# fegennari/3DWorld

Measured on NVIDIA H100. Metric: height cells/s @8192^2 8-octave domain-warp, higher is better.
Workload: dtype f32

## Files before the change

### 3dworld_b200/csrc/tw_heightgen.cu

```cuda
#include "tw_internal.h"
#include <unordered_map>
#include <vector>
#include <algorithm>
#include "tw_noise.cuh"
#include "tw_noise2.cuh"
#include <stdlib.h>

namespace {

constexpr int F_TABLE = TW_F_TABLE_SIZE;

__device__ __forceinline__ float sinf_lut(const float *__restrict__ tab, float v) {
	return (v < 0.0f) ? -__ldg(tab + (tw_x86_f2i(TW_SSCALE*(-v))&(TW_TSIZE-1))) : __ldg(tab + (tw_x86_f2i(TW_SSCALE*v)&(TW_TSIZE-1)));
}
__device__ __forceinline__ float cosf_lut(const float *__restrict__ tab, float v) {
	return __ldg(tab + TW_TSIZE + (tw_x86_f2i(TW_SSCALE*fabsf(v))&(TW_TSIZE-1)));
}
__device__ __forceinline__ float smin(float a, float b) {return (b < a) ? b : a;}
__device__ __forceinline__ float smax(float a, float b) {return (a < b) ? b : a;}

struct PostParams {
	tw_hmap_params h;
	int   shape;
	int   need_postproc;
// ... 68 lines not shown
	int   gen_shape;
	float4 oct[9];
	float xy_scale;
	float hmap_scale;
	float freq_last, rsum_last;
};

template<bool SIMPLEX, int SHAPE>
__device__ __forceinline__ float gen_noise(float xv, float yv, const NoiseParams &N) {
	float zval = 0.0f;
#pragma unroll 1
	for (int i = 0; i < N.octaves; ++i) {
		float4 const o = N.oct[i];
		float const px = o.x*xv + o.y, py = o.x*yv + o.z;
		float noise = SIMPLEX ? twn::simplex2(px, py) : twn::perlin2(px, py);
		if (SHAPE == 1) {noise = (float)((double)fabsf(noise) - 0.40);}
		if (SHAPE == 2) {noise = (float)(0.45 - (double)fabsf(noise));}
		zval = __fmaf_rn(o.w, noise, zval);
	}
	return zval;
}

template<bool SIMPLEX, bool WARP, int SHAPE>
__device__ __forceinline__ float get_noise_zval(float xval, float yval, const NoiseParams &N, const PostParams &P) {
	float xv = N.xy_scale*xval, yv = N.xy_scale*yval;
	if (WARP) {
		float const scale = 0.2f;
		float const dx1 = gen_noise<SIMPLEX, SHAPE>((float)((double)xv + 0.0), (float)((double)yv + 0.0), N);
		float const dy1 = gen_noise<SIMPLEX, SHAPE>((float)((double)xv + 5.2), (float)((double)yv + 1.3), N);
		float const wx = xv + scale*dx1, wy = yv + scale*dy1;
		float const dx2 = gen_noise<SIMPLEX, SHAPE>((float)((double)wx + 1.7), (float)((double)wy + 9.2), N);
		float const dy2 = gen_noise<SIMPLEX, SHAPE>((float)((double)wx + 8.3), (float)((double)wy + 2.8), N);
		xv += scale*dx2; yv += scale*dy2;
	}
	float z = gen_noise<SIMPLEX, SHAPE>(xv, yv, N);
	if (P.need_postproc) {z = postproc_noise_zval(z, P.h);}
	return z*N.hmap_scale;
}

template<bool SIMPLEX, bool WARP, int SHAPE>
__global__ void __launch_bounds__(256)
noise_grid_kernel(float *__restrict__ out, unsigned nx, unsigned ny, unsigned y_off, float mx0_single, float my0_single, const float2 *__restrict__ tile_origins,
	NoiseParams N, PostParams P, const float *__restrict__ sin_tab, unsigned *__restrict__ mm)
{
	unsigned const x = blockIdx.x*blockDim.x + threadIdx.x, y = y_off + blockIdx.y*blockDim.y + threadIdx.y, tile = blockIdx.z;
	float mx0 = mx0_single, my0 = my0_single;
	if (tile_origins) {float2 const o = __ldg(tile_origins + tile); mx0 = o.x; my0 = o.y;}
	float z = 0.0f;
	bool const valid = (x < nx && y < ny);
	if (valid) {
		float const xval = ((float)x*P.mdx + mx0)*P.dx_inv, yval = ((float)y*P.mdy + my0)*P.dy_inv;
		z = get_noise_zval<SIMPLEX, WARP, SHAPE>(xval, yval, N, P);
		float smx = 0.0f, smy = 0.0f;
		if (P.enable_glaciate && P.sine_on) {
			smx = P.sm_scale*cosf_lut(sin_tab, ((float)x*P.mdx + mx0)*P.dx_inv*P.sm_freq);
			smy = cosf_lut(sin_tab, ((float)y*P.mdy + my0)*P.dy_inv*P.sm_freq);
		}
		z = glaciate_and_bias(z, smx, smy, xval, yval, P, sin_tab);
		out[(size_t)tile*nx*ny + (size_t)y*nx + x] = z;
	}
	if (mm) {block_minmax(valid ? z : INFINITY, valid ? z : -INFINITY, mm + 2*tile);}
}

#ifndef TW_NOISE2_MIN_BLOCKS
#define TW_NOISE2_MIN_BLOCKS 2
#endif
#ifndef TW_NOISE2_PERSISTENT
#define TW_NOISE2_PERSISTENT 1
#endif
#ifndef TW_NOISE2_THREADS
#define TW_NOISE2_THREADS 512
#endif
#ifndef TW_NOISE2_BLOCK_CELLS
#define TW_NOISE2_BLOCK_CELLS 2048
#endif
static_assert(TW_NOISE2_BLOCK_CELLS % (2*TW_NOISE2_THREADS) == 0, "a block walks whole chunks of 2 cells per thread");
__device__ __forceinline__ bool noise_lattice_in_range(float2 xv, float2 yv, const NoiseParams &N) {
	float const bx = (fabsf(xv.x) + fabsf(yv.x))*N.freq_last + N.rsum_last, by = (fabsf(xv.y) + fabsf(yv.y))*N.freq_last + N.rsum_last;
	return (bx < 2097152.0f && by < 2097152.0f);
}

template<bool SIMPLEX, bool WARP> __host__ __device__ constexpr bool noise2_hash() {return SIMPLEX && WARP && TW_SIMPLEX_HASH_TABLE;}
template<bool HASH> __host__ __device__ constexpr int lut_entries() {return twn2::SIMPLEX_LUT_N + (HASH ? twn2::SIMPLEX_HASH_N : 0);}

template<bool SIMPLEX, int SHAPE, bool HASH>
__device__ __forceinline__ float2 gen_noise2(float2 xv, float2 yv, const NoiseParams &N, unsigned L) {
	float2 zval = make_float2(0.0f, 0.0f);
	if (noise_lattice_in_range(xv, yv, N)) {
#pragma unroll 1
		for (int i = 0; i < N.octaves; ++i) {
			float4 const o = N.oct[i];
			float2 const px = twn2::add2(twn2::mul2(xv, o.x), o.y), py = twn2::add2(twn2::mul2(yv, o.x), o.z);
			float2 noise = SIMPLEX ? ((TW_SIMPLEX_LUT > 0) ? twn2::simplex2_lut<HASH>(px, py, L) : twn2::simplex2(px, py)) : ((TW_SIMPLEX_LUT > 0) ? twn2::perlin2_lut(px, py, L) : twn2::perlin2(px, py));
			if (SHAPE == 1) {noise = make_float2((float)((double)fabsf(noise.x) - 0.40), (float)((double)fabsf(noise.y) - 0.40));}
			if (SHAPE == 2) {noise = make_float2((float)(0.45 - (double)fabsf(noise.x)), (float)(0.45 - (double)fabsf(noise.y)));}
			zval = twn2::fma2(noise, o.w, zval);
		}
	}
	else {zval = make_float2(gen_noise<SIMPLEX, SHAPE>(xv.x, yv.x, N), gen_noise<SIMPLEX, SHAPE>(xv.y, yv.y, N));}
	return zval;
}

#ifndef TW_NOISE2_DUAL
#define TW_NOISE2_DUAL 0
#endif
template<bool SIMPLEX, int SHAPE, bool HASH>
__device__ __forceinline__ void gen_noise2_dual(float2 xa, float2 ya, float2 xb, float2 yb, const NoiseParams &N, unsigned L, float2 &za, float2 &zb) {
	if (TW_SIMPLEX_LUT > 0 && noise_lattice_in_range(xa, ya, N) && noise_lattice_in_range(xb, yb, N)) {
		float2 zva = make_float2(0.0f, 0.0f), zvb = make_float2(0.0f, 0.0f);
#pragma unroll 1
		for (int i = 0; i < N.octaves; ++i) {
			float4 const o = N.oct[i];
			float const f = o.x, rx = o.y, ry = o.z, mag = o.w;
			float2 const pxa = twn2::add2(twn2::mul2(xa, f), rx), pya = twn2::add2(twn2::mul2(ya, f), ry);
			float2 const pxb = twn2::add2(twn2::mul2(xb, f), rx), pyb = twn2::add2(twn2::mul2(yb, f), ry);
			float2 na = SIMPLEX ? twn2::simplex2_lut<HASH>(pxa, pya, L) : twn2::perlin2_lut(pxa, pya, L);
			float2 nb = SIMPLEX ? twn2::simplex2_lut<HASH>(pxb, pyb, L) : twn2::perlin2_lut(pxb, pyb, L);
			if (SHAPE == 1) {na = make_float2((float)((double)fabsf(na.x) - 0.40), (float)((double)fabsf(na.y) - 0.40)); nb = make_float2((float)((double)fabsf(nb.x) - 0.40), (float)((double)fabsf(nb.y) - 0.40));}
			if (SHAPE == 2) {na = make_float2((float)(0.45 - (double)fabsf(na.x)), (float)(0.45 - (double)fabsf(na.y))); nb = make_float2((float)(0.45 - (double)fabsf(nb.x)), (float)(0.45 - (double)fabsf(nb.y)));}
			zva = twn2::fma2(na, mag, zva); zvb = twn2::fma2(nb, mag, zvb);
		}
		za = zva; zb = zvb;
	}
	else {za = gen_noise2<SIMPLEX, SHAPE, HASH>(xa, ya, N, L); zb = gen_noise2<SIMPLEX, SHAPE, HASH>(xb, yb, N, L);}
}

__device__ __forceinline__ float dadd(float a, double b) {return (float)((double)a + b);}

template<bool SIMPLEX, bool WARP, int SHAPE>
__global__ void __launch_bounds__(TW_NOISE2_THREADS, TW_NOISE2_MIN_BLOCKS)
noise_grid2_kernel(float *__restrict__ out, unsigned nx, unsigned ny, unsigned y_off, unsigned y_end, float mx0_single, float my0_single, const float2 *__restrict__ tile_origins,
	NoiseParams N, PostParams P, const float *__restrict__ sin_tab, unsigned *__restrict__ mm, const float4 *__restrict__ simplex_lut)
{
	constexpr bool HASH = noise2_hash<SIMPLEX, WARP>();
	unsigned L = 0;
	if (TW_SIMPLEX_LUT > 0) {
		extern __shared__ float4 lut_s[];
		for (int e = threadIdx.x; e < lut_entries<HASH>()*twn2::SIMPLEX_LUT_COPIES; e += blockDim.x) {lut_s[e] = __ldg(simplex_lut + e/twn2::SIMPLEX_LUT_COPIES);}
		__syncthreads();
		L = twn2::simplex_lut_base(lut_s, threadIdx.x);
		asm volatile("" : "+r"(L) :: "memory");
	}
	unsigned const tile = blockIdx.z;
	float mx0 = mx0_single, my0 = my0_single;
	if (tile_origins) {float2 const o = __ldg(tile_origins + tile); mx0 = o.x; my0 = o.y;}
	size_t const c_end = (size_t)y_end*nx;
	float lo = INFINITY, hi = -INFINITY;
	constexpr unsigned NCH = TW_NOISE2_BLOCK_CELLS/(2*TW_NOISE2_THREADS);
#pragma unroll 1
	for (unsigned grp = blockIdx.x; grp < P.ngroups; grp += gridDim.x) {
#pragma unroll 1
	for (unsigned ch = 0; ch < NCH; ++ch) {
	size_t const c0 = (size_t)y_off*nx + 2*(((size_t)grp*NCH + ch)*blockDim.x + threadIdx.x);
	unsigned y, x;
	if (c_end <= 0xffffffffull) {unsigned const c32 = (unsigned)c0; y = c32/nx; x = c32 - y*nx;}
	else {y = (unsigned)(c0/nx); x = (unsigned)(c0 - (size_t)y*nx);}
	unsigned const xb = (x + 1 < nx) ? x + 1 : 0, yb = (x + 1 < nx) ? y : y + 1;
	bool const skip = (x - P.skip_x0 < P.skip_w && y - P.skip_y0 < P.skip_h && xb - P.skip_x0 < P.skip_w && yb - P.skip_y0 < P.skip_h);
	bool const valid0 = (c0 < c_end) && !skip, valid1 = (c0 + 1 < c_end) && !skip;
	float z0 = 0.0f, z1 = 0.0f;
	if (valid0) {
		using namespace twn2;
		float2 const xs = make_float2((float)x, (float)xb), ys = make_float2((float)y, (float)yb);
		float2 const xval = mul2(add2(mul2(xs, P.mdx), mx0), P.dx_inv);
		float2 const yval = mul2(add2(mul2(ys, P.mdy), my0), P.dy_inv);
		float2 xv = mul2(xval, N.xy_scale), yv = mul2(yval, N.xy_scale);
		if (WARP) {
			float const scale = 0.2f;
			float2 dx1, dy1, dx2, dy2;
			if (TW_NOISE2_DUAL) {gen_noise2_dual<SIMPLEX, SHAPE, HASH>(make_float2(dadd(xv.x, 0.0), dadd(xv.y, 0.0)), make_float2(dadd(yv.x, 0.0), dadd(yv.y, 0.0)),
			                                                     make_float2(dadd(xv.x, 5.2), dadd(xv.y, 5.2)), make_float2(dadd(yv.x, 1.3), dadd(yv.y, 1.3)), N, L, dx1, dy1);}
			else {
				dx1 = gen_noise2<SIMPLEX, SHAPE, HASH>(make_float2(dadd(xv.x, 0.0), dadd(xv.y, 0.0)), make_float2(dadd(yv.x, 0.0), dadd(yv.y, 0.0)), N, L);
				dy1 = gen_noise2<SIMPLEX, SHAPE, HASH>(make_float2(dadd(xv.x, 5.2), dadd(xv.y, 5.2)), make_float2(dadd(yv.x, 1.3), dadd(yv.y, 1.3)), N, L);
			}
			float2 const wx = add2(xv, mul2(dx1, scale)), wy = add2(yv, mul2(dy1, scale));
			if (TW_NOISE2_DUAL) {gen_noise2_dual<SIMPLEX, SHAPE, HASH>(make_float2(dadd(wx.x, 1.7), dadd(wx.y, 1.7)), make_float2(dadd(wy.x, 9.2), dadd(wy.y, 9.2)),
			                                                     make_float2(dadd(wx.x, 8.3), dadd(wx.y, 8.3)), make_float2(dadd(wy.x, 2.8), dadd(wy.y, 2.8)), N, L, dx2, dy2);}
			else {
				dx2 = gen_noise2<SIMPLEX, SHAPE, HASH>(make_float2(dadd(wx.x, 1.7), dadd(wx.y, 1.7)), make_float2(dadd(wy.x, 9.2), dadd(wy.y, 9.2)), N, L);
				dy2 = gen_noise2<SIMPLEX, SHAPE, HASH>(make_float2(dadd(wx.x, 8.3), dadd(wx.y, 8.3)), make_float2(dadd(wy.x, 2.8), dadd(wy.y, 2.8)), N, L);
			}
			xv = add2(xv, mul2(dx2, scale)); yv = add2(yv, mul2(dy2, scale));
		}
		float2 const zz = gen_noise2<SIMPLEX, SHAPE, HASH>(xv, yv, N, L);
		z0 = zz.x; z1 = zz.y;
		if (P.need_postproc) {z0 = postproc_noise_zval(z0, P.h); z1 = postproc_noise_zval(z1, P.h);}
		z0 = z0*N.hmap_scale; z1 = z1*N.hmap_scale;
		float smx0 = 0.0f, smx1 = 0.0f, smy0 = 0.0f, smy1 = 0.0f;
		if (P.enable_glaciate && P.sine_on) {
			smx0 = P.sm_scale*cosf_lut(sin_tab, xval.x*P.sm_freq);
			smx1 = P.sm_scale*cosf_lut(sin_tab, xval.y*P.sm_freq);
			smy0 = cosf_lut(sin_tab, yval.x*P.sm_freq);
			smy1 = (yb == y) ? smy0 : cosf_lut(sin_tab, yval.y*P.sm_freq);
		}
		z0 = glaciate_and_bias(z0, smx0, smy0, xval.x, yval.x, P, sin_tab);
		z1 = glaciate_and_bias(z1, smx1, smy1, xval.y, yval.y, P, sin_tab);
		float *o = out + (size_t)(P.tile_perm ? __ldg(P.tile_perm + tile) : tile)*nx*ny + c0;
		if (valid1 && ((reinterpret_cast<size_t>(o) & 7) == 0)) {*reinterpret_cast<float2 *>(o) = make_float2(z0, z1);}
		else {o[0] = z0; if (valid1) {o[1] = z1;}}
	}
	lo = fminf(lo, fminf(valid0 ? z0 : INFINITY, valid1 ? z1 : INFINITY)); hi = fmaxf(hi, fmaxf(valid0 ? z0 : -INFINITY, valid1 ? z1 : -INFINITY));
	}
	}
	if (mm) {block_minmax(lo, hi, mm + 2*tile);}
}

template<bool SIMPLEX, bool WARP>
void launch_noise2(int shape, dim3 grid, dim3 block, cudaStream_t st, float *out, unsigned nx, unsigned ny, unsigned y_off, unsigned y_end, float mx0, float my0,
	const float2 *origins, const NoiseParams &N, const PostParams &P, const float *tab, unsigned *mm, const float4 *lut)
{
	size_t const lut_bytes = (TW_SIMPLEX_LUT > 0) ? (size_t)lut_entries<noise2_hash<SIMPLEX, WARP>()>()*twn2::SIMPLEX_LUT_COPIES*sizeof(float4) : 0;
	if (lut_bytes > 48*1024) {
		switch (shape) {
		case 1:  cudaFuncSetAttribute(noise_grid2_kernel<SIMPLEX, WARP, 1>, cudaFuncAttributeMaxDynamicSharedMemorySize, (int)lut_bytes); break;
		case 2:  cudaFuncSetAttribute(noise_grid2_kernel<SIMPLEX, WARP, 2>, cudaFuncAttributeMaxDynamicSharedMemorySize, (int)lut_bytes); break;
		default: cudaFuncSetAttribute(noise_grid2_kernel<SIMPLEX, WARP, 0>, cudaFuncAttributeMaxDynamicSharedMemorySize, (int)lut_bytes); break;
		}
	}
	switch (shape) {
	case 1:  noise_grid2_kernel<SIMPLEX, WARP, 1><<<grid, block, lut_bytes, st>>>(out, nx, ny, y_off, y_end, mx0, my0, origins, N, P, tab, mm, lut); break;
	case 2:  noise_grid2_kernel<SIMPLEX, WARP, 2><<<grid, block, lut_bytes, st>>>(out, nx, ny, y_off, y_end, mx0, my0, origins, N, P, tab, mm, lut); break;
	default: noise_grid2_kernel<SIMPLEX, WARP, 0><<<grid, block, lut_bytes, st>>>(out, nx, ny, y_off, y_end, mx0, my0, origins, N, P, tab, mm, lut); break;
	}
}

constexpr int PERLIN_LUT_OFFSET = lut_entries<true>();
__global__ void simplex_lut_kernel(float4 *__restrict__ lut) {
	int const k = blockIdx.x*blockDim.x + threadIdx.x;
	if (k < twn2::SIMPLEX_LUT_N) {lut[k] = twn2::simplex_lut_entry((float)k); lut[PERLIN_LUT_OFFSET + k] = twn2::perlin_lut_entry((float)k);}
	if (k < twn2::SIMPLEX_HASH_N) {lut[twn2::SIMPLEX_LUT_N + k] = twn2::simplex_hash_entry((float)k);}
}
static int ensure_simplex_lut(tw_ctx *ctx) {
	if (ctx->d_simplex_lut) return TW_OK;
	static_assert(twn2::SIMPLEX_HASH_N <= twn2::SIMPLEX_LUT_N, "simplex_lut_kernel's grid covers the gradient tables");
	TW_CUDA(ctx, cudaMalloc(&ctx->d_simplex_lut, (PERLIN_LUT_OFFSET + twn2::SIMPLEX_LUT_N)*sizeof(float4)));
	simplex_lut_kernel<<<(twn2::SIMPLEX_LUT_N + 127)/128, 128, 0, ctx->stream>>>((float4 *)ctx->d_simplex_lut);
	TW_LAUNCH_CHECK(ctx);
	return TW_OK;
}

struct SineTabParams {
	float msx, msy, ms2, mesh_scale_z_inv;
	float dx, dy, mx0, my0;
	int   start;
	unsigned nx, ny, xpitch, ypitch;
	int   sine_on; float sm_scale, sm_freq, dx_inv, dy_inv;
};

__global__ void sine_tables_kernel(float *__restrict__ Xt, float *__restrict__ Yt, const float *__restrict__ T, const float *__restrict__ sin_tab, SineTabParams S,
	const float *__restrict__ origins = nullptr, unsigned nux = 0, size_t xstride = 0, size_t ystride = 0)
{
	unsigned const i = blockIdx.x*blockDim.x + threadIdx.x, k = blockIdx.y;
	bool const is_y = origins ? (blockIdx.z >= nux) : (blockIdx.z != 0);
	if (origins) {
		if (is_y) {S.my0 = __ldg(origins + blockIdx.z); Yt += (size_t)(blockIdx.z - nux)*ystride;}
		else      {S.mx0 = __ldg(origins + blockIdx.z); Xt += (size_t)blockIdx.z*xstride;}
	}
	unsigned const n = is_y ? S.ny : S.nx;
	if (i >= n) return;
	if (k == F_TABLE) {
		if (!S.sine_on) return;
		if (!is_y) {Xt[(size_t)k*S.xpitch + i] = S.sm_scale*cosf_lut(sin_tab, ((float)i*S.dx + S.mx0)*S.dx_inv*S.sm_freq);}
		else       {Yt[(size_t)k*S.ypitch + i] = cosf_lut(sin_tab, ((float)i*S.dy + S.my0)*S.dy_inv*S.sm_freq);}
		return;
	}
	if ((int)k < S.start) return;
	float const *s = T + 5*k;
	if (!is_y) {
		float const x_mult = S.msx*s[4];
		float const x_const = S.ms2*s[4] + s[2] + x_mult*S.mx0;
		float const xmdx = x_mult*S.dx;
		Xt[(size_t)k*S.xpitch + i] = sinf_lut(sin_tab, xmdx*(float)i + x_const);
	}
	else {
		float const y_mult = S.msy*s[3], y_scale = S.mesh_scale_z_inv*s[0];
		float const y_const = S.ms2*s[3] + s[1] + y_mult*S.my0;
		float const ymdy = y_mult*S.dy;
		Yt[(size_t)k*S.ypitch + i] = y_scale*sinf_lut(sin_tab, ymdy*(float)i + y_const);
	}
}

constexpr int ST = 64;
constexpr int SK = 45;

__global__ void __launch_bounds__(256)
sine_grid_kernel(float *__restrict__ out, unsigned nx, unsigned ny, const float *__restrict__ Xt, const float *__restrict__ Yt,
	unsigned xpitch, unsigned ypitch, int start_ix, PostParams P, float mx0, float my0, const float *__restrict__ sin_tab, unsigned *__restrict__ mm, unsigned y_off,
	const uint2 *__restrict__ tile_tabs = nullptr, const float2 *__restrict__ tile_origins = nullptr, size_t xstride = 0, size_t ystride = 0,
	const unsigned *__restrict__ tile_perm = nullptr)
{
	__shared__ float Xs[SK][ST], Ys[SK][ST];
	if (tile_tabs) {
		unsigned const tz = tile_perm ? __ldg(tile_perm + blockIdx.z) : blockIdx.z;
		uint2 const tt = __ldg(tile_tabs + tz);
// ... 482 lines not shown
```

### 3dworld_b200/csrc/tw_noise2.cuh

```cuda
#pragma once
#include <cuda_runtime.h>
#include "tw_noise.cuh"

namespace twn2 {

typedef float2 f2;

__device__ __forceinline__ f2 splat(float v) {return make_float2(v, v);}
__device__ __forceinline__ f2 raw_fma(f2 a, f2 b, f2 c) {return make_float2(__fmaf_rn(a.x, b.x, c.x), __fmaf_rn(a.y, b.y, c.y));}
__device__ __forceinline__ f2 mul2(f2 a, f2 b) {return make_float2(__fmul_rn(a.x, b.x), __fmul_rn(a.y, b.y));}
__device__ __forceinline__ f2 mul2(f2 a, float b) {return mul2(a, splat(b));}
__device__ __forceinline__ f2 add2(f2 a, f2 b) {return make_float2(__fadd_rn(a.x, b.x), __fadd_rn(a.y, b.y));}
__device__ __forceinline__ f2 add2(f2 a, float b) {return add2(a, splat(b));}
__device__ __forceinline__ f2 sub2(f2 a, f2 b) {return make_float2(__fsub_rn(a.x, b.x), __fsub_rn(a.y, b.y));}
__device__ __forceinline__ f2 rsub2(float a, f2 b) {return sub2(splat(a), b);}
__device__ __forceinline__ f2 sumprod2(f2 a, f2 b, f2 c, f2 d) {return add2(mul2(a, b), mul2(c, d));}
__device__ __forceinline__ f2 sumprod2(f2 a, float b, f2 c, float d) {return sumprod2(a, splat(b), c, splat(d));}
__device__ __forceinline__ f2 fma2(f2 a, float b, f2 c) {return raw_fma(a, splat(b), c);}
__device__ __forceinline__ f2 fma2(f2 a, float b, float c) {return raw_fma(a, splat(b), splat(c));}
__device__ __forceinline__ f2 abs2(f2 a) {return make_float2(fabsf(a.x), fabsf(a.y));}
__device__ __forceinline__ f2 max0_2(f2 a) {return make_float2(fmaxf(a.x, 0.0f), fmaxf(a.y, 0.0f));}
__device__ __forceinline__ float rsub_max0(float a, float d) {float r; asm("sub.rn.sat.f32 %0, %1, %2;" : "=f"(r) : "f"(a), "f"(d)); return r;}
__device__ __forceinline__ f2 rsub_max0_2(float a, f2 d) {return make_float2(rsub_max0(a, d.x), rsub_max0(a, d.y));}
__device__ __forceinline__ f2 floor2(f2 x) {return make_float2(floorf(x.x), floorf(x.y));}

__device__ __forceinline__ f2 mod289(f2 x)  {f2 const t = floor2(mul2(x, 1.0f/289.0f)); return fma2(t, -289.0f, x);}
__device__ __forceinline__ f2 permute(f2 x) {return mod289(mul2(fma2(x, 34.0f, 1.0f), x));}
__device__ __forceinline__ f2 mod_int289(f2 a) {
	f2 const r = fma2(floor2(mul2(a, 1.0f/289.0f)), -289.0f, a);
	return make_float2((r.x >= 289.0f) ? r.x - 289.0f : r.x, (r.y >= 289.0f) ? r.y - 289.0f : r.y);
}
__device__ __forceinline__ f2 mod_int289_lazy(f2 a) {return fma2(floor2(mul2(a, 1.0f/289.0f)), -289.0f, a);}
__device__ __forceinline__ f2 fract2(f2 x) {return sub2(x, floor2(x));}
__device__ __forceinline__ f2 tinvsqrt(f2 r) {return rsub2(1.79284291400159f, mul2(r, 0.85373472095314f));}
__device__ __forceinline__ f2 mix2(f2 x, f2 y, f2 a) {return add2(x, mul2(a, sub2(y, x)));}
__device__ __forceinline__ f2 fade2(f2 t) {
	f2 const t3 = mul2(mul2(t, t), t);
	return mul2(t3, add2(mul2(t, add2(mul2(t, 6.0f), -15.0f)), 10.0f));
}

__device__ __forceinline__ f2 simplex2(f2 vx, f2 vy) {
	float const Cx = 0.211324865405187f, Cy = 0.366025403784439f, Cz = -0.577350269189626f, Cw = 0.024390243902439f;
	f2 const s = add2(mul2(vx, Cy), mul2(vy, Cy));
	f2 ix = floor2(add2(vx, s)), iy = floor2(add2(vy, s));
	f2 const t = add2(mul2(ix, Cx), mul2(iy, Cx));
	f2 const x0x = add2(sub2(vx, ix), t), x0y = add2(sub2(vy, iy), t);
	f2 const i1x = make_float2((x0x.x > x0y.x) ? 1.0f : 0.0f, (x0x.y > x0y.y) ? 1.0f : 0.0f);
	f2 const i1y = rsub2(1.0f, i1x);
	f2 const x12x = sub2(add2(x0x, Cx), i1x), x12y = sub2(add2(x0y, Cx), i1y), x12z = add2(x0x, Cz), x12w = add2(x0y, Cz);
	ix = mod_int289(ix); iy = mod_int289(iy);
	f2 const q0 = permute(iy), q1 = permute(add2(iy, i1y)), q2 = permute(add2(iy, 1.0f));
	f2 const p0 = permute(add2(q0, ix)), p1 = permute(add2(add2(q1, ix), i1x)), p2 = permute(add2(add2(q2, ix), 1.0f));
	f2 m0 = max0_2(rsub2(0.5f, add2(mul2(x0x, x0x), mul2(x0y, x0y))));
	f2 m1 = max0_2(rsub2(0.5f, add2(mul2(x12x, x12x), mul2(x12y, x12y))));
	f2 m2 = max0_2(rsub2(0.5f, add2(mul2(x12z, x12z), mul2(x12w, x12w))));
	m0 = mul2(m0, m0); m1 = mul2(m1, m1); m2 = mul2(m2, m2);
	m0 = mul2(m0, m0); m1 = mul2(m1, m1); m2 = mul2(m2, m2);
	f2 const t0 = mul2(p0, Cw), t1 = mul2(p1, Cw), t2 = mul2(p2, Cw);
	f2 const X0 = fma2(sub2(t0, floor2(t0)), 2.0f, -1.0f), X1 = fma2(sub2(t1, floor2(t1)), 2.0f, -1.0f), X2 = fma2(sub2(t2, floor2(t2)), 2.0f, -1.0f);
	f2 const h0 = add2(abs2(X0), -0.5f), h1 = add2(abs2(X1), -0.5f), h2 = add2(abs2(X2), -0.5f);
	f2 const a0 = sub2(X0, floor2(add2(X0, 0.5f))), a1 = sub2(X1, floor2(add2(X1, 0.5f))), a2 = sub2(X2, floor2(add2(X2, 0.5f)));
	m0 = mul2(m0, tinvsqrt(add2(mul2(a0, a0), mul2(h0, h0))));
	m1 = mul2(m1, tinvsqrt(add2(mul2(a1, a1), mul2(h1, h1))));
	m2 = mul2(m2, tinvsqrt(add2(mul2(a2, a2), mul2(h2, h2))));
	f2 const gx = add2(mul2(a0, x0x), mul2(h0, x0y)), gy = add2(mul2(a1, x12x), mul2(h1, x12y)), gz = add2(mul2(a2, x12z), mul2(h2, x12w));
	return mul2(add2(add2(mul2(m0, gx), mul2(m1, gy)), mul2(m2, gz)), 130.0f);
}

#ifndef TW_SIMPLEX_LUT
#define TW_SIMPLEX_LUT 3
#endif
constexpr int SIMPLEX_LUT_COPIES = 8;
constexpr int LUT3D_N = 580;
constexpr int SIMPLEX_LUT_N = (TW_SIMPLEX_LUT >= 3) ? 580 : 291;

__device__ __forceinline__ float4 simplex_lut_entry(float k) {
	float const Cw = 0.024390243902439f;
	float const pk = twn::permute(k);
	float const gi = (TW_SIMPLEX_LUT >= 3) ? pk : k;
	float const X = twn::two_f_minus_1(twn::fract(gi*Cw));
	float const h = fabsf(X) - 0.5f, a0 = X - floorf(X + 0.5f);
	float const n = 1.79284291400159f - 0.85373472095314f*(a0*a0 + h*h);
	return make_float4(a0, h, n, pk);
}

#ifndef TW_LUT_DENORM
#define TW_LUT_DENORM 1
#endif
#ifndef TW_HASH_Q1_ARITH
#define TW_HASH_Q1_ARITH 0
#endif
constexpr unsigned SIMPLEX_LUT_MAGIC_BITS = 0x4B400000u;
constexpr unsigned LUT_ENTRY_BYTES = 16u*SIMPLEX_LUT_COPIES;

#define TW_SIMPLEX_HASH_TABLE (TW_SIMPLEX_LUT >= 3 && TW_LUT_DENORM && !TW_HASH_Q1_ARITH)
constexpr int SIMPLEX_HASH_N = TW_SIMPLEX_HASH_TABLE ? 291 : 0;
constexpr unsigned SIMPLEX_HASH_OFFSET = SIMPLEX_LUT_N*LUT_ENTRY_BYTES;
__device__ __forceinline__ float4 simplex_hash_entry(float k) {
	float const pk = twn::permute(k);
	return make_float4(pk, pk + 1.0f, twn::permute(k + 1.0f) + 1.0f, 0.0f);
}
__device__ __forceinline__ unsigned simplex_lut_base(const float4 *lut_s, unsigned lane) {
	unsigned const a = (unsigned)__cvta_generic_to_shared(lut_s) + (lane & (SIMPLEX_LUT_COPIES - 1))*16u;
	return TW_LUT_DENORM ? a : a - SIMPLEX_LUT_MAGIC_BITS;
}
__device__ __forceinline__ f2 lut_offsets(f2 k, unsigned Lb) {
	if (TW_LUT_DENORM) {return raw_fma(k, splat(__uint_as_float(LUT_ENTRY_BYTES)), splat(__uint_as_float(Lb)));}
	return fma2(k, 16.0f*SIMPLEX_LUT_COPIES, 12582912.0f);
}
__device__ __forceinline__ unsigned lut_addr(unsigned Lb, float off) {return TW_LUT_DENORM ? __float_as_uint(off) : Lb + __float_as_uint(off);}
__device__ __forceinline__ float4 lut_load4(unsigned Lb, float off) {
	float4 v; asm("ld.shared.v4.f32 {%0, %1, %2, %3}, [%4];" : "=f"(v.x), "=f"(v.y), "=f"(v.z), "=f"(v.w) : "r"(lut_addr(Lb, off)));
	return v;
}
__device__ __forceinline__ float lut_load_w_addr(unsigned addr) {
	float v; asm("ld.shared.f32 %0, [%1+12];" : "=f"(v) : "r"(addr));
	return v;
}
__device__ __forceinline__ float lut_load_w_addr_next(unsigned addr) {
	float v; asm("ld.shared.f32 %0, [%1+140];" : "=f"(v) : "r"(addr));
	return v;
}
__device__ __forceinline__ float lut_load_w(unsigned Lb, float off) {return lut_load_w_addr(lut_addr(Lb, off));}
template<unsigned OFF> __device__ __forceinline__ float lut_load_f32(unsigned addr) {
	float v; asm("ld.shared.f32 %0, [%1+%2];" : "=f"(v) : "r"(addr), "n"(OFF));
	return v;
}

__device__ __forceinline__ void simplex_hash_args(f2 ix, f2 iy, f2 i1y, unsigned Lb, f2 &p0, f2 &p1, f2 &p2) {
	constexpr unsigned H = SIMPLEX_HASH_OFFSET;
	f2 const j0 = lut_offsets(iy, Lb);
	f2 const j1 = raw_fma(i1y, splat(__uint_as_float(LUT_ENTRY_BYTES - 4)), j0);
	unsigned const ja = __float_as_uint(j0.x), jb = __float_as_uint(j0.y), j1a = __float_as_uint(j1.x), j1b = __float_as_uint(j1.y);
	p0 = add2(make_float2(lut_load_f32<H>(ja), lut_load_f32<H>(jb)), ix);
	p1 = add2(make_float2(lut_load_f32<H + 4>(j1a), lut_load_f32<H + 4>(j1b)), ix);
	p2 = add2(make_float2(lut_load_f32<H + 8>(ja), lut_load_f32<H + 8>(jb)), ix);
}

template<bool HASH>
__device__ __forceinline__ f2 simplex2_lut(f2 vx, f2 vy, unsigned Lb) {
	static_assert(!HASH || TW_SIMPLEX_HASH_TABLE, "the hash table exists at level 3 with the denormal addressing only");
	float const Cx = 0.211324865405187f, Cy = 0.366025403784439f, Cz = -0.577350269189626f;
	f2 const s = sumprod2(vx, Cy, vy, Cy);
	f2 ix = floor2(add2(vx, s)), iy = floor2(add2(vy, s));
	f2 const t = sumprod2(ix, Cx, iy, Cx);
	f2 const x0x = add2(sub2(vx, ix), t), x0y = add2(sub2(vy, iy), t);
	f2 const i1x = make_float2((x0x.x > x0y.x) ? 1.0f : 0.0f, (x0x.y > x0y.y) ? 1.0f : 0.0f);
	f2 const i1y = rsub2(1.0f, i1x);
	f2 const x12x = sub2(add2(x0x, Cx), i1x), x12y = sub2(add2(x0y, Cx), i1y), x12z = add2(x0x, Cz), x12w = add2(x0y, Cz);
	f2 p0, p1, p2;
	if constexpr (HASH) {simplex_hash_args(mod_int289_lazy(ix), mod_int289_lazy(iy), i1y, Lb, p0, p1, p2);}
	else {
#if TW_SIMPLEX_LUT >= 2
	ix = mod_int289_lazy(ix); iy = mod_int289_lazy(iy);
	f2 const j0 = lut_offsets(iy, Lb);
	unsigned const ja = lut_addr(Lb, j0.x), jb = lut_addr(Lb, j0.y);
	static_assert(LUT_ENTRY_BYTES == 128, "lut_load_w_addr_next hard-codes the entry pitch");
	f2 const q0 = make_float2(lut_load_w_addr(ja), lut_load_w_addr(jb));
#if TW_HASH_Q1_ARITH && TW_SIMPLEX_LUT >= 3
#elif TW_LUT_DENORM
	f2 const j1 = raw_fma(i1y, splat(__uint_as_float(LUT_ENTRY_BYTES)), j0);
	f2 const q1 = make_float2(lut_load_w_addr(__float_as_uint(j1.x)), lut_load_w_addr(__float_as_uint(j1.y)));
#else
	f2 const q1 = make_float2(lut_load_w_addr(ja + ((x0x.x > x0y.x) ? 0u : LUT_ENTRY_BYTES)), lut_load_w_addr(jb + ((x0x.y > x0y.y) ? 0u : LUT_ENTRY_BYTES)));
#endif
	f2 const q2 = make_float2(lut_load_w_addr_next(ja), lut_load_w_addr_next(jb));
#else
	ix = mod_int289(ix); iy = mod_int289(iy);
	f2 const q0 = permute(iy), q1 = permute(add2(iy, i1y)), q2 = permute(add2(iy, 1.0f));
#endif
#if TW_SIMPLEX_LUT >= 3 && TW_HASH_Q1_ARITH
	p0 = add2(q0, ix); f2 const dq = sub2(q2, q0), e1 = add2(p0, 1.0f); p2 = add2(e1, dq); p1 = raw_fma(i1y, add2(dq, -1.0f), e1);
#elif TW_SIMPLEX_LUT >= 3
	p0 = add2(q0, ix); p1 = add2(add2(q1, ix), i1x); p2 = add2(add2(q2, ix), 1.0f);
#else
	p0 = permute(add2(q0, ix)); p1 = permute(add2(add2(q1, ix), i1x)); p2 = permute(add2(add2(q2, ix), 1.0f));
#endif
	}
	f2 m0 = rsub_max0_2(0.5f, sumprod2(x0x, x0x, x0y, x0y));
	f2 m1 = rsub_max0_2(0.5f, sumprod2(x12x, x12x, x12y, x12y));
	f2 m2 = rsub_max0_2(0.5f, sumprod2(x12z, x12z, x12w, x12w));
	m0 = mul2(m0, m0); m1 = mul2(m1, m1); m2 = mul2(m2, m2);
	m0 = mul2(m0, m0); m1 = mul2(m1, m1); m2 = mul2(m2, m2);
	f2 const k0 = lut_offsets(p0, Lb), k1 = lut_offsets(p1, Lb), k2 = lut_offsets(p2, Lb);
	float4 const g0a = lut_load4(Lb, k0.x), g0b = lut_load4(Lb, k0.y), g1a = lut_load4(Lb, k1.x), g1b = lut_load4(Lb, k1.y), g2a = lut_load4(Lb, k2.x), g2b = lut_load4(Lb, k2.y);
	m0 = make_float2(m0.x*g0a.z, m0.y*g0b.z); m1 = make_float2(m1.x*g1a.z, m1.y*g1b.z); m2 = make_float2(m2.x*g2a.z, m2.y*g2b.z);
	f2 const gx = make_float2(g0a.x*x0x.x  + g0a.y*x0y.x,  g0b.x*x0x.y  + g0b.y*x0y.y);
	f2 const gy = make_float2(g1a.x*x12x.x + g1a.y*x12y.x, g1b.x*x12x.y + g1b.y*x12y.y);
	f2 const gz = make_float2(g2a.x*x12z.x + g2a.y*x12w.x, g2b.x*x12z.y + g2b.y*x12w.y);
	return mul2(add2(add2(mul2(m0, gx), mul2(m1, gy)), mul2(m2, gz)), 130.0f);
}

__device__ __forceinline__ void perlin2_corner(f2 ix, f2 iy, f2 &gx, f2 &gy) {
	f2 const i = permute(add2(permute(ix), iy));
	float const c41 = 1.0f/41.0f;
	f2 const q0 = mul2(i, c41);
	f2 const q = fma2(fma2(q0, -41.0f, i), c41, q0);
	f2 const g = fma2(fract2(q), 2.0f, -1.0f);
	gy = add2(abs2(g), -0.5f);
	gx = sub2(g, floor2(add2(g, 0.5f)));
	f2 const n = tinvsqrt(add2(mul2(gx, gx), mul2(gy, gy)));
	gx = mul2(gx, n); gy = mul2(gy, n);
}

__device__ __forceinline__ f2 perlin2(f2 Px, f2 Py) {
	f2 const flx = floor2(Px), fly = floor2(Py);
	f2 const frx = sub2(Px, flx), fry = sub2(Py, fly);
	f2 const Pfz = add2(frx, -1.0f), Pfw = add2(fry, -1.0f);
	f2 const Pix = mod_int289(flx), Piy = mod_int289(fly), Piz = mod_int289(add2(flx, 1.0f)), Piw = mod_int289(add2(fly, 1.0f));
	f2 g00x, g00y, g10x, g10y, g01x, g01y, g11x, g11y;
	perlin2_corner(Pix, Piy, g00x, g00y);
	perlin2_corner(Piz, Piy, g10x, g10y);
	perlin2_corner(Pix, Piw, g01x, g01y);
	perlin2_corner(Piz, Piw, g11x, g11y);
	f2 const n00 = add2(mul2(g00x, frx), mul2(g00y, fry));
	f2 const n10 = add2(mul2(g10x, Pfz), mul2(g10y, fry));
	f2 const n01 = add2(mul2(g01x, frx), mul2(g01y, Pfw));
	f2 const n11 = add2(mul2(g11x, Pfz), mul2(g11y, Pfw));
	f2 const fdx = fade2(frx), fdy = fade2(fry);
	f2 const nx0 = mix2(n00, n10, fdx), nx1 = mix2(n01, n11, fdx);
	return mul2(mix2(nx0, nx1, fdy), 2.3f);
}

__device__ __forceinline__ float4 perlin_lut_entry(float k) {
	float const pk = twn::permute(k);
	float const g = twn::two_f_minus_1(twn::fract(twn::div41_small((TW_SIMPLEX_LUT >= 3) ? pk : k)));
	float gy = fabsf(g) - 0.5f, gx = g - floorf(g + 0.5f);
	float const n = twn::tinvsqrt(gx*gx + gy*gy);
	gx *= n; gy *= n;
	return make_float4(gx, gy, 0.0f, pk);
}

__device__ __forceinline__ f2 perlin2_lut(f2 Px, f2 Py, unsigned Lb) {
	f2 const flx = floor2(Px), fly = floor2(Py);
	f2 const frx = sub2(Px, flx), fry = sub2(Py, fly);
	f2 const Pfz = add2(frx, -1.0f), Pfw = add2(fry, -1.0f);
	f2 const Pix = mod_int289_lazy(flx), Piy = mod_int289_lazy(fly), Piz = mod_int289_lazy(add2(flx, 1.0f)), Piw = mod_int289_lazy(add2(fly, 1.0f));
	f2 const jx = lut_offsets(Pix, Lb), jz = lut_offsets(Piz, Lb);
	f2 const qx = make_float2(lut_load_w(Lb, jx.x), lut_load_w(Lb, jx.y)), qz = make_float2(lut_load_w(Lb, jz.x), lut_load_w(Lb, jz.y));
#if TW_SIMPLEX_LUT >= 3
	f2 const k00 = lut_offsets(add2(qx, Piy), Lb), k10 = lut_offsets(add2(qz, Piy), Lb), k01 = lut_offsets(add2(qx, Piw), Lb), k11 = lut_offsets(add2(qz, Piw), Lb);
#else
	f2 const k00 = lut_offsets(permute(add2(qx, Piy)), Lb), k10 = lut_offsets(permute(add2(qz, Piy)), Lb);
	f2 const k01 = lut_offsets(permute(add2(qx, Piw)), Lb), k11 = lut_offsets(permute(add2(qz, Piw)), Lb);
#endif
	float4 const a00 = lut_load4(Lb, k00.x), b00 = lut_load4(Lb, k00.y), a10 = lut_load4(Lb, k10.x), b10 = lut_load4(Lb, k10.y);
	float4 const a01 = lut_load4(Lb, k01.x), b01 = lut_load4(Lb, k01.y), a11 = lut_load4(Lb, k11.x), b11 = lut_load4(Lb, k11.y);
	f2 const n00 = make_float2(a00.x*frx.x + a00.y*fry.x, b00.x*frx.y + b00.y*fry.y);
	f2 const n10 = make_float2(a10.x*Pfz.x + a10.y*fry.x, b10.x*Pfz.y + b10.y*fry.y);
	f2 const n01 = make_float2(a01.x*frx.x + a01.y*Pfw.x, b01.x*frx.y + b01.y*Pfw.y);
	f2 const n11 = make_float2(a11.x*Pfz.x + a11.y*Pfw.x, b11.x*Pfz.y + b11.y*Pfw.y);
	f2 const fdx = fade2(frx), fdy = fade2(fry);
	f2 const nx0 = mix2(n00, n10, fdx), nx1 = mix2(n01, n11, fdx);
	return mul2(mix2(nx0, nx1, fdy), 2.3f);
}

__device__ __forceinline__ float4 simplex3_lut_entry(float k) {
	float X, Y, H;
	float const pk = twn::permute(k);
	twn::simplex3_xyh(pk, X, Y, H);
	float const sh = -twn::step(H, 0.0f);
	float Px = X + (floorf(X)*2.0f + 1.0f)*sh, Py = Y + (floorf(Y)*2.0f + 1.0f)*sh, Pz = H;
	float const n = twn::tinvsqrt(Px*Px + Py*Py + Pz*Pz);
	Px *= n; Py *= n; Pz *= n;
	return make_float4(Px, Py, Pz, pk);
}
__device__ __forceinline__ float4 perlin3_lut_entry(float k) {
// ... 63 lines not shown
```

Measured before the change: 8.369 billion.

## Store pre-scaled byte offsets in simplex hash table and restructure warp evaluation loop

The simplex hash table now holds pre-scaled byte offsets rather than permutation values. This lets the gradient lookup addresses come from one add instead of a separate lut_offsets conversion, and the hash region is now stored once instead of replicated per copy, which shrinks shared memory. The five noise evaluations of the domain warp are folded into a single rolled loop with offsets in constant memory, and the inner 8-octave loop is fully unrolled for the hash case. The aim is fewer ALU ops per octave, a smaller instruction footprint and more occupancy. The trade-off is a single-copy hash region that may cause more shared-memory bank conflicts, plus a double-precision constant-memory read in each loop iteration.

```diff
diff --git a/3dworld_b200/csrc/tw_heightgen.cu b/3dworld_b200/csrc/tw_heightgen.cu
--- a/3dworld_b200/csrc/tw_heightgen.cu
+++ b/3dworld_b200/csrc/tw_heightgen.cu
@@ -174,20 +174,28 @@
 
 template<bool SIMPLEX, bool WARP> __host__ __device__ constexpr bool noise2_hash() {return SIMPLEX && WARP && TW_SIMPLEX_HASH_TABLE;}
 template<bool HASH> __host__ __device__ constexpr int lut_entries() {return twn2::SIMPLEX_LUT_N + (HASH ? twn2::SIMPLEX_HASH_N : 0);}
+template<bool HASH> __host__ __device__ constexpr int lut_slots() {return twn2::SIMPLEX_LUT_N*twn2::SIMPLEX_LUT_COPIES + (HASH ? twn2::SIMPLEX_HASH_N*twn2::SIMPLEX_HASH_COPIES : 0);}
+
+template<bool SIMPLEX, int SHAPE, bool HASH>
+__device__ __forceinline__ float2 noise2_octave(float2 xv, float2 yv, float4 o, unsigned L, float2 zval) {
+	float2 const px = twn2::add2(twn2::mul2(xv, o.x), o.y), py = twn2::add2(twn2::mul2(yv, o.x), o.z);
+	float2 noise = SIMPLEX ? ((TW_SIMPLEX_LUT > 0) ? twn2::simplex2_lut<HASH>(px, py, L) : twn2::simplex2(px, py)) : ((TW_SIMPLEX_LUT > 0) ? twn2::perlin2_lut(px, py, L) : twn2::perlin2(px, py));
+	if (SHAPE == 1) {noise = make_float2((float)((double)fabsf(noise.x) - 0.40), (float)((double)fabsf(noise.y) - 0.40));}
+	if (SHAPE == 2) {noise = make_float2((float)(0.45 - (double)fabsf(noise.x)), (float)(0.45 - (double)fabsf(noise.y)));}
+	return twn2::fma2(noise, o.w, zval);
+}
 
 template<bool SIMPLEX, int SHAPE, bool HASH>
 __device__ __forceinline__ float2 gen_noise2(float2 xv, float2 yv, const NoiseParams &N, unsigned L) {
 	float2 zval = make_float2(0.0f, 0.0f);
-	if (noise_lattice_in_range(xv, yv, N)) {
+	bool const in_range = noise_lattice_in_range(xv, yv, N);
+	if (HASH && SHAPE == 0 && N.octaves == 8 && in_range) {
+#pragma unroll
+		for (int i = 0; i < 8; ++i) {zval = noise2_octave<SIMPLEX, SHAPE, HASH>(xv, yv, N.oct[i], L, zval);}
+	}
+	else if (in_range) {
 #pragma unroll 1
-		for (int i = 0; i < N.octaves; ++i) {
-			float4 const o = N.oct[i];
-			float2 const px = twn2::add2(twn2::mul2(xv, o.x), o.y), py = twn2::add2(twn2::mul2(yv, o.x), o.z);
-			float2 noise = SIMPLEX ? ((TW_SIMPLEX_LUT > 0) ? twn2::simplex2_lut<HASH>(px, py, L) : twn2::simplex2(px, py)) : ((TW_SIMPLEX_LUT > 0) ? twn2::perlin2_lut(px, py, L) : twn2::perlin2(px, py));
-			if (SHAPE == 1) {noise = make_float2((float)((double)fabsf(noise.x) - 0.40), (float)((double)fabsf(noise.y) - 0.40));}
-			if (SHAPE == 2) {noise = make_float2((float)(0.45 - (double)fabsf(noise.x)), (float)(0.45 - (double)fabsf(noise.y)));}
-			zval = twn2::fma2(noise, o.w, zval);
-		}
+		for (int i = 0; i < N.octaves; ++i) {zval = noise2_octave<SIMPLEX, SHAPE, HASH>(xv, yv, N.oct[i], L, zval);}
 	}
 	else {zval = make_float2(gen_noise<SIMPLEX, SHAPE>(xv.x, yv.x, N), gen_noise<SIMPLEX, SHAPE>(xv.y, yv.y, N));}
 	return zval;
@@ -218,6 +226,7 @@
 }
 
 __device__ __forceinline__ float dadd(float a, double b) {return (float)((double)a + b);}
+__constant__ double2 warp_offsets[4] = {{0.0, 0.0}, {5.2, 1.3}, {1.7, 9.2}, {8.3, 2.8}};
 
 template<bool SIMPLEX, bool WARP, int SHAPE>
 __global__ void __launch_bounds__(TW_NOISE2_THREADS, TW_NOISE2_MIN_BLOCKS)
@@ -228,7 +237,10 @@
 	unsigned L = 0;
 	if (TW_SIMPLEX_LUT > 0) {
 		extern __shared__ float4 lut_s[];
-		for (int e = threadIdx.x; e < lut_entries<HASH>()*twn2::SIMPLEX_LUT_COPIES; e += blockDim.x) {lut_s[e] = __ldg(simplex_lut + e/twn2::SIMPLEX_LUT_COPIES);}
+		constexpr int G = twn2::SIMPLEX_LUT_N*twn2::SIMPLEX_LUT_COPIES;
+		for (int e = threadIdx.x; e < lut_slots<HASH>(); e += blockDim.x) {
+			lut_s[e] = __ldg(simplex_lut + ((e < G) ? e/twn2::SIMPLEX_LUT_COPIES : twn2::SIMPLEX_LUT_N + (e - G)/twn2::SIMPLEX_HASH_COPIES));
+		}
 		__syncthreads();
 		L = twn2::simplex_lut_base(lut_s, threadIdx.x);
 		asm volatile("" : "+r"(L) :: "memory");
@@ -257,25 +269,34 @@
 		float2 const xval = mul2(add2(mul2(xs, P.mdx), mx0), P.dx_inv);
 		float2 const yval = mul2(add2(mul2(ys, P.mdy), my0), P.dy_inv);
 		float2 xv = mul2(xval, N.xy_scale), yv = mul2(yval, N.xy_scale);
+		float2 zz;
+		if (WARP && !TW_NOISE2_DUAL) {
+			float const scale = 0.2f;
+			float2 bx = xv, by = yv, d = make_float2(0.0f, 0.0f);
+#pragma unroll 1
+			for (int s = 0; s < 5; ++s) {
+				float2 sx = xv, sy = yv;
+				if (s < 4) {double2 const o = warp_offsets[s]; sx = make_float2(dadd(bx.x, o.x), dadd(bx.y, o.x)); sy = make_float2(dadd(by.x, o.y), dadd(by.y, o.y));}
+				float2 const r = gen_noise2<SIMPLEX, SHAPE, HASH>(sx, sy, N, L);
+				if (s == 1) {bx = add2(xv, mul2(d, scale)); by = add2(yv, mul2(r, scale));}
+				if (s == 3) {xv = add2(xv, mul2(d, scale)); yv = add2(yv, mul2(r, scale));}
+				d = r;
+			}
+			zz = d;
+		}
+		else {
 		if (WARP) {
 			float const scale = 0.2f;
 			float2 dx1, dy1, dx2, dy2;
-			if (TW_NOISE2_DUAL) {gen_noise2_dual<SIMPLEX, SHAPE, HASH>(make_float2(dadd(xv.x, 0.0), dadd(xv.y, 0.0)), make_float2(dadd(yv.x, 0.0), dadd(yv.y, 0.0)),
-			                                                     make_float2(dadd(xv.x, 5.2), dadd(xv.y, 5.2)), make_float2(dadd(yv.x, 1.3), dadd(yv.y, 1.3)), N, L, dx1, dy1);}
-			else {
-				dx1 = gen_noise2<SIMPLEX, SHAPE, HASH>(make_float2(dadd(xv.x, 0.0), dadd(xv.y, 0.0)), make_float2(dadd(yv.x, 0.0), dadd(yv.y, 0.0)), N, L);
-				dy1 = gen_noise2<SIMPLEX, SHAPE, HASH>(make_float2(dadd(xv.x, 5.2), dadd(xv.y, 5.2)), make_float2(dadd(yv.x, 1.3), dadd(yv.y, 1.3)), N, L);
-			}
+			gen_noise2_dual<SIMPLEX, SHAPE, HASH>(make_float2(dadd(xv.x, 0.0), dadd(xv.y, 0.0)), make_float2(dadd(yv.x, 0.0), dadd(yv.y, 0.0)),
+			                                      make_float2(dadd(xv.x, 5.2), dadd(xv.y, 5.2)), make_float2(dadd(yv.x, 1.3), dadd(yv.y, 1.3)), N, L, dx1, dy1);
 			float2 const wx = add2(xv, mul2(dx1, scale)), wy = add2(yv, mul2(dy1, scale));
-			if (TW_NOISE2_DUAL) {gen_noise2_dual<SIMPLEX, SHAPE, HASH>(make_float2(dadd(wx.x, 1.7), dadd(wx.y, 1.7)), make_float2(dadd(wy.x, 9.2), dadd(wy.y, 9.2)),
-			                                                     make_float2(dadd(wx.x, 8.3), dadd(wx.y, 8.3)), make_float2(dadd(wy.x, 2.8), dadd(wy.y, 2.8)), N, L, dx2, dy2);}
-			else {
-				dx2 = gen_noise2<SIMPLEX, SHAPE, HASH>(make_float2(dadd(wx.x, 1.7), dadd(wx.y, 1.7)), make_float2(dadd(wy.x, 9.2), dadd(wy.y, 9.2)), N, L);
-				dy2 = gen_noise2<SIMPLEX, SHAPE, HASH>(make_float2(dadd(wx.x, 8.3), dadd(wx.y, 8.3)), make_float2(dadd(wy.x, 2.8), dadd(wy.y, 2.8)), N, L);
-			}
+			gen_noise2_dual<SIMPLEX, SHAPE, HASH>(make_float2(dadd(wx.x, 1.7), dadd(wx.y, 1.7)), make_float2(dadd(wy.x, 9.2), dadd(wy.y, 9.2)),
+			                                      make_float2(dadd(wx.x, 8.3), dadd(wx.y, 8.3)), make_float2(dadd(wy.x, 2.8), dadd(wy.y, 2.8)), N, L, dx2, dy2);
 			xv = add2(xv, mul2(dx2, scale)); yv = add2(yv, mul2(dy2, scale));
 		}
-		float2 const zz = gen_noise2<SIMPLEX, SHAPE, HASH>(xv, yv, N, L);
+		zz = gen_noise2<SIMPLEX, SHAPE, HASH>(xv, yv, N, L);
+		}
 		z0 = zz.x; z1 = zz.y;
 		if (P.need_postproc) {z0 = postproc_noise_zval(z0, P.h); z1 = postproc_noise_zval(z1, P.h);}
 		z0 = z0*N.hmap_scale; z1 = z1*N.hmap_scale;
@@ -302,7 +323,7 @@
 void launch_noise2(int shape, dim3 grid, dim3 block, cudaStream_t st, float *out, unsigned nx, unsigned ny, unsigned y_off, unsigned y_end, float mx0, float my0,
 	const float2 *origins, const NoiseParams &N, const PostParams &P, const float *tab, unsigned *mm, const float4 *lut)
 {
-	size_t const lut_bytes = (TW_SIMPLEX_LUT > 0) ? (size_t)lut_entries<noise2_hash<SIMPLEX, WARP>()>()*twn2::SIMPLEX_LUT_COPIES*sizeof(float4) : 0;
+	size_t const lut_bytes = (TW_SIMPLEX_LUT > 0) ? (size_t)lut_slots<noise2_hash<SIMPLEX, WARP>()>()*sizeof(float4) : 0;
 	if (lut_bytes > 48*1024) {
 		switch (shape) {
 		case 1:  cudaFuncSetAttribute(noise_grid2_kernel<SIMPLEX, WARP, 1>, cudaFuncAttributeMaxDynamicSharedMemorySize, (int)lut_bytes); break;
diff --git a/3dworld_b200/csrc/tw_noise2.cuh b/3dworld_b200/csrc/tw_noise2.cuh
--- a/3dworld_b200/csrc/tw_noise2.cuh
+++ b/3dworld_b200/csrc/tw_noise2.cuh
@@ -95,10 +95,11 @@
 
 #define TW_SIMPLEX_HASH_TABLE (TW_SIMPLEX_LUT >= 3 && TW_LUT_DENORM && !TW_HASH_Q1_ARITH)
 constexpr int SIMPLEX_HASH_N = TW_SIMPLEX_HASH_TABLE ? 291 : 0;
+constexpr int SIMPLEX_HASH_COPIES = 1;
 constexpr unsigned SIMPLEX_HASH_OFFSET = SIMPLEX_LUT_N*LUT_ENTRY_BYTES;
 __device__ __forceinline__ float4 simplex_hash_entry(float k) {
-	float const pk = twn::permute(k);
-	return make_float4(pk, pk + 1.0f, twn::permute(k + 1.0f) + 1.0f, 0.0f);
+	unsigned const p0 = (unsigned)twn::permute(k), p1 = (unsigned)twn::permute(k + 1.0f);
+	return make_float4(__uint_as_float(LUT_ENTRY_BYTES*p0), __uint_as_float(LUT_ENTRY_BYTES*(p0 + 1)), __uint_as_float(LUT_ENTRY_BYTES*(p1 + 1)), 0.0f);
 }
 __device__ __forceinline__ unsigned simplex_lut_base(const float4 *lut_s, unsigned lane) {
 	unsigned const a = (unsigned)__cvta_generic_to_shared(lut_s) + (lane & (SIMPLEX_LUT_COPIES - 1))*16u;
@@ -127,14 +128,16 @@
 	return v;
 }
 
-__device__ __forceinline__ void simplex_hash_args(f2 ix, f2 iy, f2 i1y, unsigned Lb, f2 &p0, f2 &p1, f2 &p2) {
-	constexpr unsigned H = SIMPLEX_HASH_OFFSET;
-	f2 const j0 = lut_offsets(iy, Lb);
-	f2 const j1 = raw_fma(i1y, splat(__uint_as_float(LUT_ENTRY_BYTES - 4)), j0);
+__device__ __forceinline__ void simplex_hash_offsets(f2 ix, f2 iy, f2 i1y, unsigned Lb, f2 &k0, f2 &k1, f2 &k2) {
+	constexpr unsigned H = SIMPLEX_HASH_OFFSET, PITCH = 16u*SIMPLEX_HASH_COPIES;
+	unsigned const base = Lb - (threadIdx.x & (SIMPLEX_LUT_COPIES - 1))*16u;
+	f2 const j0 = raw_fma(iy, splat(__uint_as_float(PITCH)), splat(__uint_as_float(base)));
+	f2 const j1 = raw_fma(i1y, splat(__uint_as_float(PITCH - 4)), j0);
 	unsigned const ja = __float_as_uint(j0.x), jb = __float_as_uint(j0.y), j1a = __float_as_uint(j1.x), j1b = __float_as_uint(j1.y);
-	p0 = add2(make_float2(lut_load_f32<H>(ja), lut_load_f32<H>(jb)), ix);
-	p1 = add2(make_float2(lut_load_f32<H + 4>(j1a), lut_load_f32<H + 4>(j1b)), ix);
-	p2 = add2(make_float2(lut_load_f32<H + 8>(ja), lut_load_f32<H + 8>(jb)), ix);
+	f2 const bx = lut_offsets(ix, Lb);
+	k0 = add2(make_float2(lut_load_f32<H>(ja), lut_load_f32<H>(jb)), bx);
+	k1 = add2(make_float2(lut_load_f32<H + 4>(j1a), lut_load_f32<H + 4>(j1b)), bx);
+	k2 = add2(make_float2(lut_load_f32<H + 8>(ja), lut_load_f32<H + 8>(jb)), bx);
 }
 
 template<bool HASH>
@@ -148,9 +151,10 @@
 	f2 const i1x = make_float2((x0x.x > x0y.x) ? 1.0f : 0.0f, (x0x.y > x0y.y) ? 1.0f : 0.0f);
 	f2 const i1y = rsub2(1.0f, i1x);
 	f2 const x12x = sub2(add2(x0x, Cx), i1x), x12y = sub2(add2(x0y, Cx), i1y), x12z = add2(x0x, Cz), x12w = add2(x0y, Cz);
+	f2 k0, k1, k2;
+	if constexpr (HASH) {simplex_hash_offsets(mod_int289_lazy(ix), mod_int289_lazy(iy), i1y, Lb, k0, k1, k2);}
+	else {
 	f2 p0, p1, p2;
-	if constexpr (HASH) {simplex_hash_args(mod_int289_lazy(ix), mod_int289_lazy(iy), i1y, Lb, p0, p1, p2);}
-	else {
 #if TW_SIMPLEX_LUT >= 2
 	ix = mod_int289_lazy(ix); iy = mod_int289_lazy(iy);
 	f2 const j0 = lut_offsets(iy, Lb);
@@ -176,13 +180,13 @@
 #else
 	p0 = permute(add2(q0, ix)); p1 = permute(add2(add2(q1, ix), i1x)); p2 = permute(add2(add2(q2, ix), 1.0f));
 #endif
+	k0 = lut_offsets(p0, Lb); k1 = lut_offsets(p1, Lb); k2 = lut_offsets(p2, Lb);
 	}
 	f2 m0 = rsub_max0_2(0.5f, sumprod2(x0x, x0x, x0y, x0y));
 	f2 m1 = rsub_max0_2(0.5f, sumprod2(x12x, x12x, x12y, x12y));
 	f2 m2 = rsub_max0_2(0.5f, sumprod2(x12z, x12z, x12w, x12w));
 	m0 = mul2(m0, m0); m1 = mul2(m1, m1); m2 = mul2(m2, m2);
 	m0 = mul2(m0, m0); m1 = mul2(m1, m1); m2 = mul2(m2, m2);
-	f2 const k0 = lut_offsets(p0, Lb), k1 = lut_offsets(p1, Lb), k2 = lut_offsets(p2, Lb);
 	float4 const g0a = lut_load4(Lb, k0.x), g0b = lut_load4(Lb, k0.y), g1a = lut_load4(Lb, k1.x), g1b = lut_load4(Lb, k1.y), g2a = lut_load4(Lb, k2.x), g2b = lut_load4(Lb, k2.y);
 	m0 = make_float2(m0.x*g0a.z, m0.y*g0b.z); m1 = make_float2(m1.x*g1a.z, m1.y*g1b.z); m2 = make_float2(m2.x*g2a.z, m2.y*g2b.z);
 	f2 const gx = make_float2(g0a.x*x0x.x  + g0a.y*x0y.x,  g0b.x*x0x.y  + g0b.y*x0y.y);
```

Result: faster. 8.781 billion (median of 6 runs) (+4.9%).
